# kabkabm/defensegan

Hardware: NVIDIA H100
Metric: reconstructed images/sec at R=10,L=200 (higher is better)
Workload: dtype f16

## Files before the change

defensegan_b200/csrc/dgan_api.cu:

```cuda
#include <algorithm>
#include <cmath>
#include <cstdio>
#include <cstring>
#include <functional>
#include <memory>
#include <new>

#include "common.cuh"
#include "kernels_simt.cuh"
#include "kernels_tc.cuh"
#include "kernels_tc2.cuh"
#include "kernels_vjp.cuh"
#include "kernels_measured.cuh"
#include "kernels_measured_csr.cuh"
#include "kernels_measured_conv.cuh"
#include "kernels_prune.cuh"
#include "kernels_adam.cuh"
#include "kernels_sparse_dev.cuh"

namespace dgan {

static thread_local std::string g_last_error;
void set_error(const std::string& msg) { g_last_error = msg; }

// ... 215 lines not shown
  int n_bands = 0;
  int n_blocks = 0;
  size_t fwd_smem = 0, bwd_smem = 0;
};

}

using namespace dgan;

struct dgan_ctx {
  dgan_desc desc;
  Widths wd{};
  int H = 0, W = 0, C = 0, hwc = 0;
  std::vector<GemmLayer> layers;
  FinalLayer fin;
  std::vector<void*> allocs;
  int64_t macs_per_row = 0;
  int64_t last_launches = 0;
  int64_t launches = 0;
  TcState tc;
  std::vector<TcDir> tc_dirs;
  std::vector<TcDir> tc_jvp_dirs;
  std::vector<TcDir> tc_w_dirs;
  bool profile = false;
  int n_rows_cur = 0;
  struct LoopGraph {
    const void* ws; int batch, rec_rr, rec_iters, decay_lr, weighted, measured, csr_nnz; float rec_lr, momentum;
    std::vector<int> prune;
    cudaGraphExec_t exec; int64_t kernels;
    int adam = 0; float beta1 = 0.f, beta2 = 0.f, eps = 0.f;
    float huber = 0.f;
    std::vector<int> conv;
    int prior = 0; float z_prior = 0.f;
    int sdev = 0; float sdev_l1 = 0.f, sdev_step = 0.f;
    bool same_key(const LoopGraph& o) const {
      return ws == o.ws && batch == o.batch && rec_rr == o.rec_rr && rec_iters == o.rec_iters && decay_lr == o.decay_lr &&
             weighted == o.weighted && measured == o.measured && csr_nnz == o.csr_nnz && rec_lr == o.rec_lr &&
             momentum == o.momentum && prune == o.prune && adam == o.adam && beta1 == o.beta1 && beta2 == o.beta2 &&
             eps == o.eps && huber == o.huber && conv == o.conv && prior == o.prior && z_prior == o.z_prior &&
             sdev == o.sdev && sdev_l1 == o.sdev_l1 && sdev_step == o.sdev_step;
    }
  };
  std::vector<LoopGraph> graphs;
  cudaStream_t cap_stream = nullptr;
  int64_t last_enqueues = 0;
  struct ProfRec { int kind; cudaEvent_t a, b; };
// ... 853 lines not shown
static int image_loss_finish(dgan_ctx* c, const Workspace& w, cudaStream_t s) {
  return loss_finish(c, w, w.loss_part, w.n_loss_parts, w.loss_stride_n, w.loss_stride_b, 1.0f / (float)c->hwc, s);
}

static int plan_all(dgan_ctx* c, int n_rows) {
  if (c->desc.precision != DGAN_PREC_FP16) return 0;
  const int n_mpairs = (int)align_up((size_t)std::max(n_rows, 1), 2 * kRowTile) / (2 * kRowTile);
  int rc;
  for (TcDir& t : c->tc_dirs)
    if ((rc = tc2_get_schedule(t, n_mpairs, c->tc.num_sms / 2, &c->allocs))) return rc;
  return 0;
}

static int plan_pass(dgan_ctx* c, int n_rows, TcPass pass) {
  if (c->desc.precision != DGAN_PREC_FP16) return 0;
  int rc;
  std::vector<TcDir>& have = pass == TC_PASS_TANGENT ? c->tc_jvp_dirs : c->tc_w_dirs;
  if (have.empty()) {
    std::vector<TcDir> dirs = tc_directions(&c->desc, pass);
    for (TcDir& t : dirs) {
      if ((rc = tc_dir_supported(t))) return rc;
      for (const TcDir& p : c->tc_dirs)
        if (p.ld == t.ld && p.col0 == t.col0) { t.w = p.w; t.tm_b = p.tm_b; }
    }
    have = std::move(dirs);
  }
  const int n_mpairs = (int)align_up((size_t)std::max(n_rows, 1), 2 * kRowTile) / (2 * kRowTile);
  for (TcDir& t : have)
    if ((rc = tc2_get_schedule(t, n_mpairs, c->tc.num_sms / 2, &c->allocs))) return rc;
  return 0;
}

static int check_ws(dgan_ctx* c, int n_rows, void* ws, size_t ws_bytes, Workspace* out, bool weighted = false, int m = 0,
                    int csr_nnz = -1, bool adam = false, const ConvGeom* conv = nullptr, bool sdev = false) {
  if (ws == nullptr) { set_error("workspace is NULL"); return DGAN_ERR_WORKSPACE; }
  if (((uintptr_t)ws & 1023) != 0) { set_error("workspace must be 1024-byte aligned"); return DGAN_ERR_WORKSPACE; }
  int rc;
  const bool wpass = weighted && !sdev;
  if ((rc = plan_all(c, n_rows))) return rc;
  if (wpass && (rc = plan_pass(c, n_rows, TC_PASS_WEIGHTED))) return rc;
  *out = carve(c, n_rows, ws, nullptr, weighted, m, csr_nnz, false, nullptr, adam, conv, sdev);
  if (out->bytes > ws_bytes) {
    set_error("workspace too small: need " + std::to_string(out->bytes) + " bytes, got " + std::to_string(ws_bytes) +
              (sdev ? (m > 0 ? " (dgan_workspace_bytes_measured_sparse_dev)" : " (dgan_workspace_bytes_sparse_dev)")
               : conv != nullptr ? " (dgan_workspace_bytes_measured_conv)"
               : adam ? (m > 0 ? " (dgan_workspace_bytes_measured_adam)" : " (dgan_workspace_bytes_adam)")
// ... 1412 lines not shown
    flops_per_launch_out[k] = 2.0 * h->kind_macs_per_row[k] * (double)h->n_rows_cur;
  }
  for (auto& r : h->prof) {
    DGAN_CUDA_CHECK(cudaEventSynchronize(r.b));
    float ms = 0.f;
    DGAN_CUDA_CHECK(cudaEventElapsedTime(&ms, r.a, r.b));
    if (r.kind >= 0 && r.kind < nk) { ms_out[r.kind] += ms; launches_out[r.kind]++; }
    cudaEventDestroy(r.a); cudaEventDestroy(r.b);
  }
  h->prof.clear();
  return DGAN_OK;
}

static int check_plans_impl(const dgan_desc* d, int n_rows, int n_pairs, int mutate, TcPass pass) {
  using namespace dgan;
  if (d == nullptr || n_rows <= 0 || n_pairs <= 0) { set_error("invalid argument"); return DGAN_ERR_INVALID_ARG; }
  const int n_pad = ((n_rows + 2 * kRowTile - 1) / (2 * kRowTile)) * 2 * kRowTile, n_mpairs = n_pad / (2 * kRowTile);
  Widths wd;
  if (int rc = padded_widths(d, &wd)) return rc;
  const std::string wide_target = pass == TC_PASS_TANGENT ? "Generator.3.jvp" : pass == TC_PASS_WEIGHTED ? "last.fwd.w" : "Generator.3.fwd";
  for (const TcDir& dr : tc_directions(d, pass)) {
    if (int rc = tc_dir_supported(dr)) return rc;
    Tc2Plan plan;
    int rc = tc2_plan(dr.N, dr.K, dr.tab, dr.h_grid, dr.w_grid, dr.max_acc, 0, dr.epi, dr.out_bytes, n_mpairs, n_pairs, &plan);
    if (rc) { set_error(dr.name + ": " + dgan_last_error()); return rc; }
    const bool narrow = (mutate == 12 || mutate == 13) && dr.name == "last.bwd";
    const bool wide = mutate != 0 && mutate != 12 && mutate != 13 && dr.name == wide_target;
    if ((narrow || wide) && plan.stream_m.size() > 40) {
      auto mma = [&](size_t i, auto f) { TcMmaRec m = TcMmaRec::decode(plan.stream_m[i]); f(m); plan.stream_m[i] = m.encode(); };
      auto producer = [&](size_t i, auto f) { TcProducerRec p = TcProducerRec::decode(plan.stream_p[i]); f(p); plan.stream_p[i] = p.encode(); };
      auto every_mma = [&](auto f) { for (size_t i = 0; i < plan.stream_m.size(); ++i) mma(i, f); };
      switch (mutate) {
        case 1: mma(20, [](TcMmaRec& m) {
                  TcOp op = TcOp::decode(m.ops[0]);
                  op.first ^= 1u;
                  m.ops[0] = op.encode();
                });
                break;
        case 2: mma(20, [](TcMmaRec& m) {
                  for (uint32_t j = 1; j < m.maxb; ++j)
                    if (m.ops[j] != m.ops[0]) { std::swap(m.ops[0], m.ops[j]); break; }
                });
                break;
        case 3: producer(20, [](TcProducerRec& p) { p.tile[0] ^= 1u; }); break;
        case 4: producer(20, [](TcProducerRec& p) { p.pix[0] ^= 1u; }); break;
        case 5: producer(20, [](TcProducerRec& p) { p.kc ^= 1u; }); break;
        case 6: plan.eitems[0] = -1; break;
// ... 12 lines not shown
        case 13: producer(20, [](TcProducerRec& p) { p.kc |= 1u; }); break;
        case 14: mma(20, [](TcMmaRec& m) {
                   for (uint32_t j = 0; j < m.maxb; ++j) m.ops[j] = TC2_PAD_OP;
                 });
                 break;
        case 15: {
                   bool done = false;
                   for (size_t i = 20; i < plan.stream_m.size() && !done; ++i)
                     mma(i, [&](TcMmaRec& m) {
                       for (uint32_t j = 0; j < m.n_rounds * m.maxb && !done; ++j)
                         if (TcOp::decode(m.ops[j]).slot == (uint32_t)TC2_ZERO_SLOT) {
                           m.ops[j] = (uint8_t)TcOp::First::put(m.ops[j], 1u);
                           done = true;
                         }
                     });
                   break;
                 }
        default: break;
      }
    }
    std::string err;
    if ((rc = tc2_check_plan(dr.N, dr.K, dr.tab, n_mpairs, dr.epi, dr.out_bytes, plan, &err))) { set_error(dr.name + ": " + err); return rc; }
    if (mutate != 0) continue;
    for (const Tc2Kind& k : kTc2Kinds) {
      if (k.n != dr.N || k.ksub != plan.ksub || k.epi != dr.epi || k.out_bytes != dr.out_bytes || k.maxb == plan.maxb) continue;
      Tc2Plan forced;
      if ((rc = tc2_plan(dr.N, dr.K, dr.tab, dr.h_grid, dr.w_grid, dr.max_acc, k.maxb, dr.epi, dr.out_bytes, n_mpairs, n_pairs, &forced))) {
        set_error(dr.name + " (" + std::to_string(k.maxb) + " slots): " + dgan_last_error());
        return rc;
      }
      if ((rc = tc2_check_plan(dr.N, dr.K, dr.tab, n_mpairs, dr.epi, dr.out_bytes, forced, &err))) {
        set_error(dr.name + " (" + std::to_string(k.maxb) + " slots): " + err);
        return rc;
      }
    }
  }
  return 0;
}

int dgan_debug_check_plans(const dgan_desc* d, int n_rows, int n_pairs, int mutate) {
  return check_plans_impl(d, n_rows, n_pairs, mutate, TC_PASS_PROJ);
}

int dgan_debug_check_tangent_plans(const dgan_desc* d, int n_rows, int n_pairs, int mutate) {
  return check_plans_impl(d, n_rows, n_pairs, mutate, TC_PASS_TANGENT);
}

int dgan_debug_check_weighted_plans(const dgan_desc* d, int n_rows, int n_pairs, int mutate) {
  return check_plans_impl(d, n_rows, n_pairs, mutate, TC_PASS_WEIGHTED);
}


int dgan_debug_force_slots(dgan_handle h, int dir, int maxb) {
  if (h == nullptr || h->desc.precision != DGAN_PREC_FP16 || maxb < 0) { set_error("invalid argument"); return DGAN_ERR_INVALID_ARG; }
  if (dir < 0 || dir >= (int)h->tc_dirs.size()) { set_error("layer-direction out of range"); return DGAN_ERR_INVALID_ARG; }
  TcDir& d = h->tc_dirs[(size_t)dir];
  if (maxb > 0 && !tc2_has_kind(d.N, maxb, tc2_ksub(d.K), d.epi, d.out_bytes)) {
    set_error("no kernel instantiation with " + std::to_string(maxb) + " accumulator slots per round for this layer-direction");
    return DGAN_ERR_UNSUPPORTED;
  }
  d.force_maxb = maxb;
  d.by_mpairs.clear();
  for (auto& g : h->graphs) cudaGraphExecDestroy(g.exec);
  h->graphs.clear();
  return DGAN_OK;
}

int dgan_debug_slot_choices(dgan_handle h, int dir, int* out, int max_n) {
  if (h == nullptr || h->desc.precision != DGAN_PREC_FP16 || out == nullptr) return -1;
  if (dir < 0 || dir >= (int)h->tc_dirs.size()) return -1;
  const TcDir& d = h->tc_dirs[(size_t)dir];
  int n = 0;
  for (const Tc2Kind& k : kTc2Kinds)
    if (k.n == d.N && k.ksub == tc2_ksub(d.K) && k.epi == d.epi && k.out_bytes == d.out_bytes && n < max_n) out[n++] = k.maxb;
  return n;
}

#ifdef DGAN_PROBE
int dgan_debug_probe_read(unsigned long long* out) {
  if (cudaDeviceSynchronize() != cudaSuccess) return -1;
  if (cudaMemcpyFromSymbol(out, dgan::g_tc2_probe, sizeof(dgan::g_tc2_probe)) != cudaSuccess) return -1;
  static unsigned long long zeros[48 * 160 * dgan::TC2_PROBE_WORDS];
  if (cudaMemcpyToSymbol(dgan::g_tc2_probe, zeros, sizeof(zeros)) != cudaSuccess) return -1;
  return 0;
}
// ... 6 lines not shown
  const int n_pad = ((n_rows + 2 * kRowTile - 1) / (2 * kRowTile)) * 2 * kRowTile, n_mpairs = n_pad / (2 * kRowTile);
  Widths wd;
  if (padded_widths(d, &wd) != 0) return -1;
  std::string out = "direction | N | K | window (h x w, stride) | items | slots | steps | MMAs | staged MB | busiest pair / mean load"
                    " | zero-tile MMA % | MMAs per round | busiest pair: est. tensor us | busiest pair: est. us | k16 MMAs"
                    " | epilogue/output\n";
  auto epi_name = [](int epi) {
    switch (epi) {
      case EPI_BIAS_RELU: return "bias_relu";
      case EPI_BIAS: return "bias";
      case EPI_MASK: return "mask";
      case EPI_FINAL_SIGMOID1: return "final_sigmoid";
      case EPI_FINAL_TANH3: return "final_tanh";
      default: return "none";
    }
  };
  double total = 0.0;
  const std::vector<TcDir> dirs = tc_directions(d);
  for (size_t di = 0; di < dirs.size(); ++di) {
    const TcDir& dr = dirs[di];
    Tc2Plan plan;
    const bool forced = (int)di == force_dir;
    const int rc = tc2_plan(dr.N, dr.K, dr.tab, dr.h_grid, dr.w_grid, dr.max_acc, forced ? force_maxb : 0, dr.epi, dr.out_bytes,
                            n_mpairs, n_pairs, &plan, forced ? force_shape : nullptr);
    if (rc) return -1;
    char line[320];
    const double mb = (double)plan.n_bytes / 1e6;
    total += mb;
    snprintf(line, sizeof line, "%s | %d | %d | %dx%d, %dx%d | %zu | %d | %lld | %lld | %.1f | %.3f | %.1f | %d | %.1f | %.1f | %lld | %s/f%d\n",
             dr.name.c_str(), dr.N, dr.K, plan.shape[0], plan.shape[1], plan.shape[2], plan.shape[3],
             plan.hdrs.size() * (size_t)n_mpairs, plan.n_slots, plan.n_steps, plan.n_mma, mb, plan.load_max / std::max(plan.load_mean, 1.0),
             100.0 * (double)plan.n_pad / (double)std::max(plan.n_mma, 1LL), plan.maxb, plan.op_ns_max / 1e3,
             plan.load_max / 1e3, plan.n_mma * plan.ksub, epi_name(dr.epi), 8 * dr.out_bytes);
    out += line;
  }
  char line[64];
  snprintf(line, sizeof line, "total staged MB per L-step | %.1f\n", total);
  out += line;
  const int n = (int)std::min(out.size(), (size_t)buf_len - 1);
  memcpy(buf, out.data(), (size_t)n);
  buf[n] = 0;
  return n;
}

int dgan_debug_plan_stats_slots(const dgan_desc* d, int n_rows, int n_pairs, int force_dir, int force_maxb, char* buf, int buf_len) {
  return plan_stats_impl(d, n_rows, n_pairs, force_dir, force_maxb, nullptr, buf, buf_len);
}

int dgan_debug_plan_stats_window(const dgan_desc* d, int n_rows, int n_pairs, int force_dir, int force_maxb, int wh, int ww,
                                 int sy, int sx, char* buf, int buf_len) {
  const int shape[4] = {wh, ww, sy, sx};
  return plan_stats_impl(d, n_rows, n_pairs, force_dir, force_maxb, shape, buf, buf_len);
}

int dgan_debug_plan_issue_stats(const dgan_desc* d, int n_rows, int n_pairs, char* buf, int buf_len) {
  using namespace dgan;
  if (d == nullptr || n_rows <= 0 || n_pairs <= 0 || buf == nullptr || buf_len <= 0) { set_error("invalid argument"); return -1; }
  const int n_pad = ((n_rows + 2 * kRowTile - 1) / (2 * kRowTile)) * 2 * kRowTile, n_mpairs = n_pad / (2 * kRowTile);
  Widths wd;
  if (padded_widths(d, &wd) != 0) return -1;
  std::string out = "direction | slots | k16 MMAs issued | zero-tile k16 MMAs skipped | busiest pair: est. tensor us, issued\n";
  for (const TcDir& dr : tc_directions(d)) {
    Tc2Plan plan;
    if (tc2_plan(dr.N, dr.K, dr.tab, dr.h_grid, dr.w_grid, dr.max_acc, 0, dr.epi, dr.out_bytes, n_mpairs, n_pairs, &plan)) return -1;
    char line[200];
    snprintf(line, sizeof line, "%s | %d | %lld | %lld | %.1f\n", dr.name.c_str(), plan.maxb, plan.n_issued * plan.ksub,
             (plan.n_mma - plan.n_issued) * plan.ksub, plan.op_ns_issued_max / 1e3);
    out += line;
  }
  const int n = (int)std::min(out.size(), (size_t)buf_len - 1);
  memcpy(buf, out.data(), (size_t)n);
  buf[n] = 0;
  return n;
}

int dgan_debug_padded_widths(const dgan_desc* d, int* out) {
  using namespace dgan;
  if (d == nullptr || out == nullptr) { set_error("invalid argument"); return DGAN_ERR_INVALID_ARG; }
  Widths w;
  if (int rc = padded_widths(d, &w)) return rc;
  out[0] = w.latent; out[1] = w.c4; out[2] = w.c2; out[3] = w.c1;
  return 0;
}

static int workspace_layout_impl(dgan_handle h, int n_rows, char* buf, int buf_len, bool weighted, int m = 0,
                                 int csr_nnz = -1) {
  if (h == nullptr || n_rows <= 0 || buf == nullptr || buf_len <= 0) { set_error("invalid argument"); return -1; }
// ... 109 lines not shown
```

defensegan_b200/csrc/kernels_tc2.cuh:

```cuda
#pragma once
#include "kernels_tc.cuh"
#include "tc_records.cuh"

namespace dgan {

constexpr int TC2_SMEM_MAX = 232448;
constexpr int TC2_TILE_BYTES = 128 * 128;
constexpr int TC2_BUF_COLS = 256;
constexpr int TC2_CONSUMERS = 256;
constexpr int TC2_THREADS = TC2_CONSUMERS + 128;
constexpr int TC2_PRODUCER_REGS = 40, TC2_CONSUMER_REGS = 232;
constexpr int TC2_STORE_ROWS = 16;

constexpr int TC2_MAX_PAIRS = 80;
struct Tc2Heads {
  uint32_t off[TC2_MAX_PAIRS + 1];
};

struct __align__(16) TcItem2 {
  uint16_t q[16];
  uint32_t n_acc;
};
static_assert(sizeof(TcItem2) == 48 && offsetof(TcItem2, n_acc) == 32, "the kernel's item loads");

// ... 819 lines not shown
      if (probe_steps != 0) atomicAdd(&g_tc2_probe[key][blockIdx.x][14], (unsigned long long)((unsigned)clock64() - probe_h0));
      atomicAdd(&g_tc2_probe[key][blockIdx.x][0], (unsigned long long)(clock64() - probe_t_go));
      atomicAdd(&g_tc2_probe[key][blockIdx.x][1], 1ull);
      atomicAdd(&g_tc2_probe[key][blockIdx.x][2], (unsigned long long)(probe_t_go - probe_t_entry));
      atomicAdd(&g_tc2_probe[key][blockIdx.x][4], (unsigned long long)(probe_t_entry - probe_t_start));
      g_tc2_probe[key][blockIdx.x][5] = probe_g_start;
      g_tc2_probe[key][blockIdx.x][6] = probe_gtime();
    }
  }
#endif
  ptx::cluster_sync();
}

struct Tc2Schedule {
  TcItem2* items = nullptr;
  TcRec* stream_p = nullptr;
  TcRec* stream_m = nullptr;
  Tc2Heads heads{};
  int* eitems = nullptr;
  int n_slots = 0, n_pairs = 0;
  int maxb = 1;
};
static uint32_t tc2_box_k(int K) { return tc2_ksub(K) == 4 ? 64u : 16u; }
struct TcDir {
  std::string name, kind;
  int N = 0, K = 0, P_in = 0, P_out = 0, n_tiles = 0;
  PairTable tab;
  int h_grid = 0, w_grid = 0;
  int max_acc = 1;
  int epi = EPI_NONE, out_bytes = 2, bias_pstride = 0;
  int ld = 0, col0 = 0, out_ld = 0;
  int n_real = 0;
  std::string base_kind;
  __half* w = nullptr;
  CUtensorMap tm_b{};
  int force_maxb = 0;
  std::vector<std::pair<int, Tc2Schedule>> by_mpairs;
};

static int tc2_maxb(int N) { return TC2_BUF_COLS / tc2_acc_stride(N); }

struct Tc2HostStep {
  int kc = 0, nA = 0, nB = 0, n_rounds = 0;
  int a_pix[TC2_MAX_A] = {0, 0, 0, 0};
  uint8_t b_ent[TC2_MAX_BSLOTS] = {0};
  uint8_t ops[TC2_OP_BYTES] = {0};
  int n_real = 0;
  int bytes = 0;
};
struct Tc2HostItem {
  TcItem2 hdr{};
  std::vector<Tc2HostStep> steps;
  double stage_bytes = 0.0;
  long long n_ops = 0;
  long long n_issued = 0;
};

static void tc2_build_item(const PairTable& tab, const std::vector<int>& qs, int N, int K, int max_b, int max_a,
                           int step_max_bytes, Tc2HostItem* out) {
// ... 125 lines not shown
#define DGAN_STEP_MAX_KB_N64 64
#endif
#ifndef DGAN_COST_EPI_KB
#define DGAN_COST_EPI_KB 24.0
#endif
#ifndef DGAN_COST_FIXED_KB
#define DGAN_COST_FIXED_KB 48.0
#endif
#ifndef DGAN_COST_NS_PER_KB
#define DGAN_COST_NS_PER_KB 6.8
#endif
#ifndef DGAN_COST_OP_NS
#define DGAN_COST_OP_NS 103.0
#endif
#ifndef DGAN_COST_STEP_NS
#define DGAN_COST_STEP_NS 942.0
#endif
#ifndef DGAN_COST_OP_MIN_N
#define DGAN_COST_OP_MIN_N 32
#endif
#ifndef TC2_REFINE_BUDGET
#define TC2_REFINE_BUDGET (1LL << 26)
#endif

struct Tc2Plan {
  int shape[4] = {1, 1, 1, 1};
  int n_slots = 0, n_pairs = 0;
  std::vector<TcItem2> hdrs;
  std::vector<TcRec> stream_p, stream_m;
  std::vector<uint32_t> stream_off;
  std::vector<int> eitems;
  long long n_mma = 0, n_pad = 0, n_issued = 0, n_steps = 0, n_bytes = 0;
  double load_max = 0.0, load_mean = 0.0;
  double op_ns_max = 0.0;
  double op_ns_issued_max = 0.0;
  int maxb = 1, ring_bytes = 0;
  int ksub = 4;
};

static double tc2_op_ns(int N, int ksub) {
  return DGAN_COST_OP_NS * (double)std::max(N, DGAN_COST_OP_MIN_N) / 64.0 * (double)ksub / 4.0;
}

static int tc2_search(int N, int K, const PairTable& tab, int h_grid, int w_grid, int max_acc, int force_maxb, int epi,
                      int out_bytes, int n_mpairs, int n_pairs, const int* force_shape, Tc2Plan* plan,
                      std::vector<Tc2HostItem>* best_items, std::vector<std::vector<int>>* best_lists) {
  const int max_a = TC2_MAX_A;
  const int step_kb = (N == 64 && K == 128) ? DGAN_STEP_MAX_KB_N64 : DGAN_STEP_MAX_KB;
  const int ksub = tc2_ksub(K);
  const double op_ns = tc2_op_ns(N, ksub);
  double best_cost = 1e300;
  plan->maxb = 0;
  std::vector<std::vector<int>> wins;
  for (const Tc2Kind& kind : kTc2Kinds) {
    if (kind.n != N || kind.ksub != ksub || kind.epi != epi || kind.out_bytes != out_bytes) continue;
    if (force_maxb > 0 && kind.maxb != force_maxb) continue;
    const int mb = kind.maxb, ring = tc2_ring_bytes(N, mb, ksub, epi, out_bytes);
    const int step_max = std::min((ring / 3) & ~1023, step_kb * 1024);
    for (int wh = 1; wh <= 2; ++wh)
      for (int ww = 1; ww <= 8; ++ww)
        for (int sy = 1; sy <= (wh > 1 ? 2 : 1); ++sy)
          for (int sx = 1; sx <= (ww > 1 ? 2 : 1); ++sx) {
            if (wh * ww > std::min(max_acc, mb) || wh > h_grid || ww > std::max(w_grid, 1)) continue;
            if (force_shape != nullptr && (wh != force_shape[0] || ww != force_shape[1] || sy != force_shape[2] || sx != force_shape[3])) continue;
            tc2_enumerate_windows(h_grid, std::max(w_grid, 1), wh, ww, sy, sx, &wins);
            std::vector<Tc2HostItem> items(wins.size());
            for (size_t i = 0; i < wins.size(); ++i) tc2_build_item(tab, wins[i], N, K, mb, max_a, step_max, &items[i]);
            std::vector<double> icost(items.size());
            auto cost_item = [&](const Tc2HostItem& it) {
              return DGAN_COST_NS_PER_KB / 1024.0 *
                         (it.stage_bytes + DGAN_COST_EPI_KB * 1024.0 * it.hdr.n_acc * std::max(1, N / 64) + DGAN_COST_FIXED_KB * 1024.0) +
                     op_ns * (double)it.n_ops + DGAN_COST_STEP_NS * (double)it.steps.size();
            };
            std::stable_sort(items.begin(), items.end(), [](const Tc2HostItem& l, const Tc2HostItem& r) { return l.stage_bytes > r.stage_bytes; });
            for (size_t i = 0; i < items.size(); ++i) icost[i] = cost_item(items[i]);
            const long long total = (long long)items.size() * n_mpairs;
            std::vector<double> load((size_t)n_pairs, 0.0);
            std::vector<std::vector<int>> lists((size_t)n_pairs);
            for (long long idx = 0; idx < total; ++idx) {
              size_t best = 0;
              for (size_t pr = 1; pr < (size_t)n_pairs; ++pr)
                if (load[pr] < load[best]) best = pr;
              load[best] += icost[(size_t)(idx / n_mpairs)];
              lists[best].push_back((int)idx);
            }
            auto cost_of = [&](int idx) { return icost[(size_t)(idx / n_mpairs)]; };
            long long work = 0;
            for (int iter = 0; iter < 4096 && work < TC2_REFINE_BUDGET; ++iter) {
              const size_t P = (size_t)(std::max_element(load.begin(), load.end()) - load.begin());
              double best_peak = load[P];
              size_t bq = P; int bi = -1, bj = -1;
              for (size_t Q = 0; Q < (size_t)n_pairs; ++Q) {
                if (Q == P) continue;
                work += (long long)lists[P].size() * (long long)(1 + lists[Q].size());
                for (size_t i = 0; i < lists[P].size(); ++i) {
                  const double ci = cost_of(lists[P][i]);
                  double peak = std::max(load[P] - ci, load[Q] + ci);
                  if (peak < best_peak - 1e-9) { best_peak = peak; bq = Q; bi = (int)i; bj = -1; }
                  for (size_t j = 0; j < lists[Q].size(); ++j) {
                    const double cj = cost_of(lists[Q][j]);
                    if (cj >= ci) continue;
                    peak = std::max(load[P] - ci + cj, load[Q] + ci - cj);
                    if (peak < best_peak - 1e-9) { best_peak = peak; bq = Q; bi = (int)i; bj = (int)j; }
                  }
                }
              }
              if (bi < 0) break;
              const int it_i = lists[P][(size_t)bi];
              const double ci = cost_of(it_i);
              if (bj < 0) {
                lists[P].erase(lists[P].begin() + bi);
                lists[bq].push_back(it_i);
                load[P] -= ci; load[bq] += ci;
              } else {
                const int it_j = lists[bq][(size_t)bj];
                const double cj = cost_of(it_j);
                lists[P][(size_t)bi] = it_j; lists[bq][(size_t)bj] = it_i;
                load[P] += cj - ci; load[bq] += ci - cj;
              }
            }
            for (auto& l : lists)
              std::stable_sort(l.begin(), l.end(), [&](int a, int b) { return cost_of(a) > cost_of(b); });
            const double makespan = *std::max_element(load.begin(), load.end());
            if (makespan < best_cost) {
              best_cost = makespan;
              plan->load_max = makespan;
              plan->load_mean = std::accumulate(load.begin(), load.end(), 0.0) / (double)n_pairs;
              plan->shape[0] = wh; plan->shape[1] = ww; plan->shape[2] = sy; plan->shape[3] = sx;
              plan->maxb = mb; plan->ring_bytes = ring;
              plan->op_ns_max = 0.0;
              plan->op_ns_issued_max = 0.0;
              for (size_t pr = 0; pr < lists.size(); ++pr)
                if (load[pr] == makespan) {
                  for (int idx : lists[pr]) {
                    plan->op_ns_max += op_ns * (double)items[(size_t)(idx / n_mpairs)].n_ops;
                    plan->op_ns_issued_max += op_ns * (double)items[(size_t)(idx / n_mpairs)].n_issued;
                  }
                  break;
                }
              best_items->swap(items); best_lists->swap(lists);
            }
          }
  }
  if (plan->maxb == 0) { set_error("no tensor-core kernel instantiation for this layer-direction"); return DGAN_ERR_UNSUPPORTED; }
  plan->ksub = ksub;
  return 0;
}

static int tc2_encode_streams(int N, int n_mpairs, int n_pairs, const std::vector<Tc2HostItem>& items,
                              const std::vector<std::vector<int>>& lists, Tc2Plan* plan) {
  const int max_b = plan->maxb, ring_bytes = plan->ring_bytes, ksub = plan->ksub;
  plan->n_pairs = n_pairs;
  size_t n_slots = 0;
  for (auto& l : lists) n_slots = std::max(n_slots, l.size());
  plan->n_slots = (int)n_slots;
  std::vector<int>& eitems = plan->eitems;
  eitems.assign(n_slots * (size_t)n_pairs, -1);
  std::vector<uint32_t>& stream_off = plan->stream_off;
  stream_off.assign((size_t)n_pairs + 1, 0);
  std::vector<TcRec>& stream_p = plan->stream_p;
  std::vector<TcRec>& stream_m = plan->stream_m;
  stream_p.clear(); stream_m.clear();
  long long n_mma = 0, n_pad = 0, n_issued = 0, n_steps = 0, n_bytes = 0;
  for (size_t pr = 0; pr < lists.size(); ++pr) {
    stream_off[pr] = (uint32_t)stream_m.size();
    std::vector<std::pair<int, int>> region;
    int cursor = 0;
    for (size_t k = 0; k < lists[pr].size(); ++k) {
      const int win = lists[pr][k] / n_mpairs, mp = lists[pr][k] % n_mpairs;
      if ((uint32_t)win > TcItemWindow::mask || (uint32_t)mp > TcItemMp::mask) { set_error("tensor-core schedule limits exceeded"); return DGAN_ERR_UNSUPPORTED; }
      eitems[k * (size_t)n_pairs + pr] = tc2_item_word(win, mp);
      const Tc2HostItem& itm = items[(size_t)win];
      for (size_t j = 0; j < itm.steps.size(); ++j) {
        const Tc2HostStep& hs = itm.steps[j];
        const int kb = (hs.bytes + 1023) / 1024;
        if (kb * 1024 > ring_bytes) { set_error("tensor-core step larger than the operand ring"); return DGAN_ERR_UNSUPPORTED; }
        if (cursor + kb > ring_bytes / 1024) cursor = 0;
        const int beg = cursor, end = cursor + kb;
        cursor = end;
        int dep = TC2_NSLOT;
        const int kidx = (int)region.size();
        for (int d = 1; d <= TC2_NSLOT && d <= kidx; ++d) {
          const auto& rg = region[(size_t)(kidx - d)];
          if (rg.first < end && beg < rg.second) { dep = d; break; }
        }
        if (dep == 1 && j > 0) { set_error("tensor-core step overlaps the step before it (ring too small)"); return DGAN_ERR_UNSUPPORTED; }
        region.push_back({beg, end});
        TcMmaRec m;
        m.off = (uint32_t)beg; m.nA = (uint32_t)hs.nA; m.n_rounds = (uint32_t)hs.n_rounds; m.maxb = (uint32_t)max_b; m.ksub = (uint32_t)ksub;
        m.flags = (j == 0 ? TcMmaRec::FIRST : 0u) | (j + 1 == itm.steps.size() ? TcMmaRec::LAST : 0u);
        std::copy(hs.ops, hs.ops + hs.n_rounds * max_b, m.ops);
        stream_m.push_back(m.encode());
        TcProducerRec p;
        p.off = (uint32_t)beg; p.kc = (uint32_t)hs.kc; p.nA = (uint32_t)hs.nA; p.nB = (uint32_t)hs.nB; p.dep = (uint32_t)dep; p.mp = (uint32_t)mp;
        std::copy(hs.a_pix, hs.a_pix + TC2_MAX_A, p.pix);
        std::copy(hs.b_ent, hs.b_ent + TC2_MAX_BSLOTS, p.tile);
        stream_p.push_back(p.encode());
        n_mma += hs.n_rounds * max_b; n_pad += hs.n_rounds * max_b - hs.n_real;
        n_issued += tc2_issues_zero_ops(max_b, ksub) ? hs.n_rounds * max_b : hs.n_real;
        n_steps += 1; n_bytes += 2LL * hs.nA * tc2_a_bytes(ksub) + (long long)hs.nB * tc2_b_bytes(N, ksub);
      }
    }
  }
  stream_off[(size_t)n_pairs] = (uint32_t)stream_m.size();
  plan->hdrs.resize(items.size());
  for (size_t i = 0; i < items.size(); ++i) plan->hdrs[i] = items[i].hdr;
  plan->n_mma = n_mma; plan->n_pad = n_pad; plan->n_issued = n_issued; plan->n_steps = n_steps; plan->n_bytes = n_bytes;
  return 0;
}

static int tc2_plan(int N, int K, const PairTable& tab, int h_grid, int w_grid, int max_acc, int force_maxb, int epi,
                    int out_bytes, int n_mpairs, int n_pairs, Tc2Plan* plan, const int* force_shape = nullptr) {
  std::vector<Tc2HostItem> items;
  std::vector<std::vector<int>> lists;
  const int rc = tc2_search(N, K, tab, h_grid, w_grid, max_acc, force_maxb, epi, out_bytes, n_mpairs, n_pairs, force_shape,
                            plan, &items, &lists);
  return rc ? rc : tc2_encode_streams(N, n_mpairs, n_pairs, items, lists, plan);
}

static int tc2_check_plan(int N, int K, const PairTable& tab, int n_mpairs, int epi, int out_bytes, const Tc2Plan& pl,
                          std::string* err) {
  auto fail = [&](const std::string& m) { *err = m; return DGAN_ERR_INVALID_ARG; };
  const int ksub = tc2_ksub(K), kch = K / (16 * ksub), a_bytes = tc2_a_bytes(ksub), b_tile = tc2_b_bytes(N, ksub);
  const int max_acc = pl.maxb;
  if (pl.ksub != ksub) return fail("plan's k16 MMAs per op disagree with the direction's channels");
  if (!tc2_has_kind(N, max_acc, ksub, epi, out_bytes)) return fail("no kernel instantiation with these accumulator slots per round");
  const int ring_bytes = tc2_ring_bytes(N, max_acc, ksub, epi, out_bytes);
  const size_t n_pairs = (size_t)pl.n_pairs;
  if (pl.stream_off.size() != n_pairs + 1) return fail("stream_off size");
  if (pl.stream_p.size() != pl.stream_m.size()) return fail("stream sizes differ");
  if (pl.eitems.size() != (size_t)pl.n_slots * n_pairs) return fail("eitems size");
  std::vector<int> assigned(pl.hdrs.size() * (size_t)n_mpairs, 0);
  for (const TcItem2& h : pl.hdrs) {
    if (h.n_acc < 1 || (int)h.n_acc > max_acc) return fail("window with too many accumulators");
    for (uint32_t a = 0; a < h.n_acc; ++a)
      if ((size_t)h.q[a] + 1 >= tab.off.size()) return fail("window pixel out of range");
  }
  struct Step { int beg, end; };
  for (size_t pr = 0; pr < n_pairs; ++pr) {
// ... 77 lines not shown
          for (int kc = 0; kc < kch; ++kc)
            for (int e2 = tab.off[hdr.q[a]]; e2 < tab.off[hdr.q[a] + 1]; ++e2) want.push_back({tab.pairs[e2].x * 32 + tab.pairs[e2].y, kc});
          std::vector<std::pair<int, int>> got = contrib[a];
          std::sort(want.begin(), want.end()); std::sort(got.begin(), got.end());
          if (want != got) return fail("an item's MMAs do not cover exactly its pair list");
        }
        in_item = false;
      }
    }
    if (in_item) return fail("stream ends inside an item");
    for (int kk = item_k + 1; kk < pl.n_slots; ++kk)
      if (pl.eitems[(size_t)kk * n_pairs + pr] != -1) return fail("epilogue list has an item the stream lacks");
  }
  for (int v : assigned)
    if (v != 1) return fail("an item is not assigned to any CTA pair");
  return 0;
}

static int tc2_get_schedule(TcDir& d, int n_mpairs, int n_pairs, std::vector<void*>* allocs) {
  for (auto& kv : d.by_mpairs)
    if (kv.first == n_mpairs) return 0;
  Tc2Plan plan;
  int rc;
  if ((rc = tc2_plan(d.N, d.K, d.tab, d.h_grid, d.w_grid, d.max_acc, d.force_maxb, d.epi, d.out_bytes, n_mpairs, n_pairs, &plan)))
    return rc;
  const cudaStream_t s = 0;
  Tc2Schedule sc;
  sc.maxb = plan.maxb;
  sc.n_pairs = n_pairs; sc.n_slots = plan.n_slots;
  if ((rc = tc_upload(allocs, plan.hdrs.data(), plan.hdrs.size() * sizeof(TcItem2), (void**)&sc.items, s))) return rc;
  if ((rc = tc_upload(allocs, plan.stream_p.data(), plan.stream_p.size() * sizeof(TcRec), (void**)&sc.stream_p, s))) return rc;
  if ((rc = tc_upload(allocs, plan.stream_m.data(), plan.stream_m.size() * sizeof(TcRec), (void**)&sc.stream_m, s))) return rc;
  if (n_pairs > TC2_MAX_PAIRS) { set_error("more CTA pairs than the kernel's parameter block holds"); return DGAN_ERR_UNSUPPORTED; }
  for (int pr = 0; pr <= n_pairs; ++pr) sc.heads.off[pr] = plan.stream_off[(size_t)pr];
  if ((rc = tc_upload(allocs, plan.eitems.data(), plan.eitems.size() * sizeof(int), (void**)&sc.eitems, s))) return rc;
  d.by_mpairs.push_back({n_mpairs, sc});
  return 0;
}

template <int NT, int MB, int KS, int EP, typename TOUT>
static cudaError_t tc2_optin() {
  return cudaFuncSetAttribute(tc_bsgemm2_kernel<NT, MB, KS, EP, TOUT>, cudaFuncAttributeMaxDynamicSharedMemorySize,
                              Tc2Cfg<NT, MB, KS, EP, (int)sizeof(TOUT)>::SMEM_BYTES);
}

static int tc2_optin_all() {
#define TC2_OPTIN(NT, MB, KS, EP, T) DGAN_CUDA_CHECK((tc2_optin<NT, MB, KS, EP, T>()));
// ... 36 lines not shown
```

Baseline: 2928.

## Order tensor-core work items in row bands to keep activations L2-resident

Adds a band ordering mode to the tensor-core scheduler. Work items are grouped by bands of row-tile pairs sized to fit a fixed L2 budget, and the band direction alternates between layers so a consumer starts on rows its producer just wrote. The band assignment is used only when its modeled makespan stays within a small tolerance of the LPT schedule and the input is large enough. It is meant to cut DRAM traffic for re-read activations, at the cost of slightly worse load balance and extra host-side planning.

```diff
diff --git a/defensegan_b200/csrc/dgan_api.cu b/defensegan_b200/csrc/dgan_api.cu
--- a/defensegan_b200/csrc/dgan_api.cu
+++ b/defensegan_b200/csrc/dgan_api.cu
@@ -261,6 +261,7 @@
   std::vector<TcDir> tc_dirs;
   std::vector<TcDir> tc_jvp_dirs;
   std::vector<TcDir> tc_w_dirs;
+  int tc_order = TC2_ORDER_BAND;
   bool profile = false;
   int n_rows_cur = 0;
   struct LoopGraph {
@@ -1160,6 +1161,7 @@
       if ((rc = tc_dir_supported(t))) return rc;
       for (const TcDir& p : c->tc_dirs)
         if (p.ld == t.ld && p.col0 == t.col0) { t.w = p.w; t.tm_b = p.tm_b; }
+      t.order = c->tc_order;
     }
     have = std::move(dirs);
   }
@@ -2618,7 +2620,9 @@
   for (const TcDir& dr : tc_directions(d, pass)) {
     if (int rc = tc_dir_supported(dr)) return rc;
     Tc2Plan plan;
-    int rc = tc2_plan(dr.N, dr.K, dr.tab, dr.h_grid, dr.w_grid, dr.max_acc, 0, dr.epi, dr.out_bytes, n_mpairs, n_pairs, &plan);
+    const bool rev = tc2_band_reverse(dr.ld);
+    int rc = tc2_plan(dr.N, dr.K, dr.tab, dr.h_grid, dr.w_grid, dr.max_acc, 0, dr.epi, dr.out_bytes, n_mpairs, n_pairs,
+                      dr.order, rev, &plan);
     if (rc) { set_error(dr.name + ": " + dgan_last_error()); return rc; }
     const bool narrow = (mutate == 12 || mutate == 13) && dr.name == "last.bwd";
     const bool wide = mutate != 0 && mutate != 12 && mutate != 13 && dr.name == wide_target;
@@ -2677,10 +2681,21 @@
     std::string err;
     if ((rc = tc2_check_plan(dr.N, dr.K, dr.tab, n_mpairs, dr.epi, dr.out_bytes, plan, &err))) { set_error(dr.name + ": " + err); return rc; }
     if (mutate != 0) continue;
+    Tc2Plan lpt;
+    if ((rc = tc2_plan(dr.N, dr.K, dr.tab, dr.h_grid, dr.w_grid, dr.max_acc, 0, dr.epi, dr.out_bytes, n_mpairs, n_pairs,
+                       TC2_ORDER_LPT, rev, &lpt))) {
+      set_error(dr.name + " (LPT order): " + dgan_last_error());
+      return rc;
+    }
+    if ((rc = tc2_check_plan(dr.N, dr.K, dr.tab, n_mpairs, dr.epi, dr.out_bytes, lpt, &err))) {
+      set_error(dr.name + " (LPT order): " + err);
+      return rc;
+    }
     for (const Tc2Kind& k : kTc2Kinds) {
       if (k.n != dr.N || k.ksub != plan.ksub || k.epi != dr.epi || k.out_bytes != dr.out_bytes || k.maxb == plan.maxb) continue;
       Tc2Plan forced;
-      if ((rc = tc2_plan(dr.N, dr.K, dr.tab, dr.h_grid, dr.w_grid, dr.max_acc, k.maxb, dr.epi, dr.out_bytes, n_mpairs, n_pairs, &forced))) {
+      if ((rc = tc2_plan(dr.N, dr.K, dr.tab, dr.h_grid, dr.w_grid, dr.max_acc, k.maxb, dr.epi, dr.out_bytes, n_mpairs, n_pairs,
+                         dr.order, rev, &forced))) {
         set_error(dr.name + " (" + std::to_string(k.maxb) + " slots): " + dgan_last_error());
         return rc;
       }
@@ -2716,6 +2731,22 @@
   }
   d.force_maxb = maxb;
   d.by_mpairs.clear();
+  for (auto& g : h->graphs) cudaGraphExecDestroy(g.exec);
+  h->graphs.clear();
+  return DGAN_OK;
+}
+
+int dgan_debug_force_order(dgan_handle h, int order) {
+  if (h == nullptr || h->desc.precision != DGAN_PREC_FP16 || (order != TC2_ORDER_LPT && order != TC2_ORDER_BAND)) {
+    set_error("invalid argument");
+    return DGAN_ERR_INVALID_ARG;
+  }
+  h->tc_order = order;
+  for (std::vector<TcDir>* dirs : {&h->tc_dirs, &h->tc_jvp_dirs, &h->tc_w_dirs})
+    for (TcDir& d : *dirs) {
+      d.order = order;
+      d.by_mpairs.clear();
+    }
   for (auto& g : h->graphs) cudaGraphExecDestroy(g.exec);
   h->graphs.clear();
   return DGAN_OK;
@@ -2768,7 +2799,7 @@
     Tc2Plan plan;
     const bool forced = (int)di == force_dir;
     const int rc = tc2_plan(dr.N, dr.K, dr.tab, dr.h_grid, dr.w_grid, dr.max_acc, forced ? force_maxb : 0, dr.epi, dr.out_bytes,
-                            n_mpairs, n_pairs, &plan, forced ? force_shape : nullptr);
+                            n_mpairs, n_pairs, dr.order, tc2_band_reverse(dr.ld), &plan, forced ? force_shape : nullptr);
     if (rc) return -1;
     char line[320];
     const double mb = (double)plan.n_bytes / 1e6;
@@ -2799,6 +2830,36 @@
   return plan_stats_impl(d, n_rows, n_pairs, force_dir, force_maxb, shape, buf, buf_len);
 }
 
+int dgan_debug_plan_order_stats(const dgan_desc* d, int n_rows, int n_pairs, int order, char* buf, int buf_len) {
+  using namespace dgan;
+  if (d == nullptr || n_rows <= 0 || n_pairs <= 0 || buf == nullptr || buf_len <= 0 ||
+      (order != TC2_ORDER_LPT && order != TC2_ORDER_BAND)) {
+    set_error("invalid argument");
+    return -1;
+  }
+  const int n_pad = ((n_rows + 2 * kRowTile - 1) / (2 * kRowTile)) * 2 * kRowTile, n_mpairs = n_pad / (2 * kRowTile);
+  Widths wd;
+  if (padded_widths(d, &wd) != 0) return -1;
+  std::string out = "direction | order | band row pairs | busiest pair: LPT us | busiest pair: order us | staged A MB"
+                    " | staged weight MB | unique input MB | working set MB\n";
+  for (const TcDir& dr : tc_directions(d)) {
+    Tc2Plan plan;
+    if (tc2_plan(dr.N, dr.K, dr.tab, dr.h_grid, dr.w_grid, dr.max_acc, 0, dr.epi, dr.out_bytes, n_mpairs, n_pairs, order,
+                 tc2_band_reverse(dr.ld), &plan))
+      return -1;
+    char line[240];
+    snprintf(line, sizeof line, "%s | %s | %d | %.1f | %.1f | %.1f | %.1f | %.1f | %.1f\n", dr.name.c_str(),
+             plan.order == TC2_ORDER_BAND ? (tc2_band_reverse(dr.ld) ? "band-" : "band+") : "lpt", plan.band_rows,
+             plan.load_max / 1e3, plan.load_max_order / 1e3, plan.n_bytes_a / 1e6, plan.n_bytes_b / 1e6,
+             plan.uniq_a_bytes / 1e6, plan.ws_a_bytes / 1e6);
+    out += line;
+  }
+  const int n = (int)std::min(out.size(), (size_t)buf_len - 1);
+  memcpy(buf, out.data(), (size_t)n);
+  buf[n] = 0;
+  return n;
+}
+
 int dgan_debug_plan_issue_stats(const dgan_desc* d, int n_rows, int n_pairs, char* buf, int buf_len) {
   using namespace dgan;
   if (d == nullptr || n_rows <= 0 || n_pairs <= 0 || buf == nullptr || buf_len <= 0) { set_error("invalid argument"); return -1; }
@@ -2808,7 +2869,9 @@
   std::string out = "direction | slots | k16 MMAs issued | zero-tile k16 MMAs skipped | busiest pair: est. tensor us, issued\n";
   for (const TcDir& dr : tc_directions(d)) {
     Tc2Plan plan;
-    if (tc2_plan(dr.N, dr.K, dr.tab, dr.h_grid, dr.w_grid, dr.max_acc, 0, dr.epi, dr.out_bytes, n_mpairs, n_pairs, &plan)) return -1;
+    if (tc2_plan(dr.N, dr.K, dr.tab, dr.h_grid, dr.w_grid, dr.max_acc, 0, dr.epi, dr.out_bytes, n_mpairs, n_pairs, dr.order,
+                 tc2_band_reverse(dr.ld), &plan))
+      return -1;
     char line[200];
     snprintf(line, sizeof line, "%s | %d | %lld | %lld | %.1f\n", dr.name.c_str(), plan.maxb, plan.n_issued * plan.ksub,
              (plan.n_mma - plan.n_issued) * plan.ksub, plan.op_ns_issued_max / 1e3);
diff --git a/defensegan_b200/csrc/kernels_tc2.cuh b/defensegan_b200/csrc/kernels_tc2.cuh
--- a/defensegan_b200/csrc/kernels_tc2.cuh
+++ b/defensegan_b200/csrc/kernels_tc2.cuh
@@ -1,4 +1,6 @@
 #pragma once
+#include <unordered_map>
+
 #include "kernels_tc.cuh"
 #include "tc_records.cuh"
 
@@ -865,6 +867,7 @@
   int maxb = 1;
 };
 static uint32_t tc2_box_k(int K) { return tc2_ksub(K) == 4 ? 64u : 16u; }
+enum Tc2Order { TC2_ORDER_LPT = 0, TC2_ORDER_BAND = 1 };
 struct TcDir {
   std::string name, kind;
   int N = 0, K = 0, P_in = 0, P_out = 0, n_tiles = 0;
@@ -878,6 +881,7 @@
   __half* w = nullptr;
   CUtensorMap tm_b{};
   int force_maxb = 0;
+  int order = TC2_ORDER_BAND;
   std::vector<std::pair<int, Tc2Schedule>> by_mpairs;
 };
 
@@ -1049,6 +1053,15 @@
 #ifndef TC2_REFINE_BUDGET
 #define TC2_REFINE_BUDGET (1LL << 26)
 #endif
+#ifndef TC2_BAND_L2_BYTES
+#define TC2_BAND_L2_BYTES (16 << 20)
+#endif
+#ifndef TC2_BAND_TOLERANCE
+#define TC2_BAND_TOLERANCE 0.02
+#endif
+#ifndef TC2_BAND_MIN_INPUT
+#define TC2_BAND_MIN_INPUT (9 << 20)
+#endif
 
 struct Tc2Plan {
   int shape[4] = {1, 1, 1, 1};
@@ -1058,9 +1071,14 @@
   std::vector<uint32_t> stream_off;
   std::vector<int> eitems;
   long long n_mma = 0, n_pad = 0, n_issued = 0, n_steps = 0, n_bytes = 0;
+  long long n_bytes_a = 0, n_bytes_b = 0;
+  long long uniq_a_bytes = 0;
+  long long ws_a_bytes = 0;
   double load_max = 0.0, load_mean = 0.0;
   double op_ns_max = 0.0;
   double op_ns_issued_max = 0.0;
+  int order = TC2_ORDER_LPT, band_rows = 0;
+  double load_max_order = 0.0;
   int maxb = 1, ring_bytes = 0;
   int ksub = 4;
 };
@@ -1069,9 +1087,84 @@
   return DGAN_COST_OP_NS * (double)std::max(N, DGAN_COST_OP_MIN_N) / 64.0 * (double)ksub / 4.0;
 }
 
+static double tc2_item_cost(const Tc2HostItem& it, int N, double op_ns) {
+  return DGAN_COST_NS_PER_KB / 1024.0 *
+             (it.stage_bytes + DGAN_COST_EPI_KB * 1024.0 * it.hdr.n_acc * std::max(1, N / 64) + DGAN_COST_FIXED_KB * 1024.0) +
+         op_ns * (double)it.n_ops + DGAN_COST_STEP_NS * (double)it.steps.size();
+}
+
+static int tc2_band_of(int idx, int n_mpairs, int band_rows, bool reverse) {
+  const int b = (idx % n_mpairs) / band_rows, n_bands = (n_mpairs + band_rows - 1) / band_rows;
+  return reverse ? n_bands - 1 - b : b;
+}
+
+static double tc2_assign(const std::vector<double>& icost, int n_mpairs, int n_pairs, int band_rows, bool reverse,
+                         size_t max_items, std::vector<std::vector<int>>* lists_out, std::vector<double>* load_out) {
+  const long long total = (long long)icost.size() * n_mpairs;
+  auto cost_of = [&](int idx) { return icost[(size_t)(idx / n_mpairs)]; };
+  auto band_of = [&](int idx) { return band_rows > 0 ? tc2_band_of(idx, n_mpairs, band_rows, reverse) : 0; };
+  std::vector<int> seq((size_t)total);
+  std::iota(seq.begin(), seq.end(), 0);
+  if (band_rows > 0)
+    std::stable_sort(seq.begin(), seq.end(), [&](int a, int b) {
+      return band_of(a) != band_of(b) ? band_of(a) < band_of(b) : cost_of(a) > cost_of(b);
+    });
+  std::vector<double>& load = *load_out;
+  std::vector<std::vector<int>>& lists = *lists_out;
+  load.assign((size_t)n_pairs, 0.0);
+  lists.assign((size_t)n_pairs, {});
+  const size_t cap = max_items > 0 ? max_items : (size_t)total;
+  for (int idx : seq) {
+    size_t best = (size_t)n_pairs;
+    for (size_t pr = 0; pr < (size_t)n_pairs; ++pr)
+      if (lists[pr].size() < cap && (best == (size_t)n_pairs || load[pr] < load[best])) best = pr;
+    load[best] += cost_of(idx);
+    lists[best].push_back(idx);
+  }
+  long long work = 0;
+  for (int iter = 0; iter < 4096 && work < TC2_REFINE_BUDGET; ++iter) {
+    const size_t P = (size_t)(std::max_element(load.begin(), load.end()) - load.begin());
+    double best_peak = load[P];
+    size_t bq = P; int bi = -1, bj = -1;
+    for (size_t Q = 0; Q < (size_t)n_pairs; ++Q) {
+      if (Q == P) continue;
+      work += (long long)lists[P].size() * (long long)(1 + lists[Q].size());
+      for (size_t i = 0; i < lists[P].size(); ++i) {
+        const double ci = cost_of(lists[P][i]);
+        double peak = std::max(load[P] - ci, load[Q] + ci);
+        if (lists[Q].size() < cap && peak < best_peak - 1e-9) { best_peak = peak; bq = Q; bi = (int)i; bj = -1; }
+        for (size_t j = 0; j < lists[Q].size(); ++j) {
+          const double cj = cost_of(lists[Q][j]);
+          if (cj >= ci || band_of(lists[Q][j]) != band_of(lists[P][i])) continue;
+          peak = std::max(load[P] - ci + cj, load[Q] + ci - cj);
+          if (peak < best_peak - 1e-9) { best_peak = peak; bq = Q; bi = (int)i; bj = (int)j; }
+        }
+      }
+    }
+    if (bi < 0) break;
+    const int it_i = lists[P][(size_t)bi];
+    const double ci = cost_of(it_i);
+    if (bj < 0) {
+      lists[P].erase(lists[P].begin() + bi);
+      lists[bq].push_back(it_i);
+      load[P] -= ci; load[bq] += ci;
+    } else {
+      const int it_j = lists[bq][(size_t)bj];
+      const double cj = cost_of(it_j);
+      lists[P][(size_t)bi] = it_j; lists[bq][(size_t)bj] = it_i;
+      load[P] += cj - ci; load[bq] += ci - cj;
+    }
+  }
+  for (auto& l : lists)
+    std::stable_sort(l.begin(), l.end(), [&](int a, int b) {
+      return band_of(a) != band_of(b) ? band_of(a) < band_of(b) : cost_of(a) > cost_of(b);
+    });
+  return *std::max_element(load.begin(), load.end());
+}
+
 static int tc2_search(int N, int K, const PairTable& tab, int h_grid, int w_grid, int max_acc, int force_maxb, int epi,
-                      int out_bytes, int n_mpairs, int n_pairs, const int* force_shape, Tc2Plan* plan,
-                      std::vector<Tc2HostItem>* best_items, std::vector<std::vector<int>>* best_lists) {
+                      int out_bytes, int n_mpairs, int n_pairs, int order, bool reverse, const int* force_shape,
+                      Tc2Plan* plan, std::vector<Tc2HostItem>* best_items, std::vector<std::vector<int>>* best_lists) {
   const int max_a = TC2_MAX_A;
   const int step_kb = (N == 64 && K == 128) ? DGAN_STEP_MAX_KB_N64 : DGAN_STEP_MAX_KB;
   const int ksub = tc2_ksub(K);
@@ -1079,6 +1172,7 @@
   double best_cost = 1e300;
   plan->maxb = 0;
   std::vector<std::vector<int>> wins;
+  std::vector<double> best_load;
   for (const Tc2Kind& kind : kTc2Kinds) {
     if (kind.n != N || kind.ksub != ksub || kind.epi != epi || kind.out_bytes != out_bytes) continue;
     if (force_maxb > 0 && kind.maxb != force_maxb) continue;
@@ -1093,84 +1187,68 @@
             tc2_enumerate_windows(h_grid, std::max(w_grid, 1), wh, ww, sy, sx, &wins);
             std::vector<Tc2HostItem> items(wins.size());
             for (size_t i = 0; i < wins.size(); ++i) tc2_build_item(tab, wins[i], N, K, mb, max_a, step_max, &items[i]);
+            std::stable_sort(items.begin(), items.end(), [](const Tc2HostItem& l, const Tc2HostItem& r) { return l.stage_bytes > r.stage_bytes; });
             std::vector<double> icost(items.size());
-            auto cost_item = [&](const Tc2HostItem& it) {
-              return DGAN_COST_NS_PER_KB / 1024.0 *
-                         (it.stage_bytes + DGAN_COST_EPI_KB * 1024.0 * it.hdr.n_acc * std::max(1, N / 64) + DGAN_COST_FIXED_KB * 1024.0) +
-                     op_ns * (double)it.n_ops + DGAN_COST_STEP_NS * (double)it.steps.size();
-            };
-            std::stable_sort(items.begin(), items.end(), [](const Tc2HostItem& l, const Tc2HostItem& r) { return l.stage_bytes > r.stage_bytes; });
-            for (size_t i = 0; i < items.size(); ++i) icost[i] = cost_item(items[i]);
-            const long long total = (long long)items.size() * n_mpairs;
-            std::vector<double> load((size_t)n_pairs, 0.0);
-            std::vector<std::vector<int>> lists((size_t)n_pairs);
-            for (long long idx = 0; idx < total; ++idx) {
-              size_t best = 0;
-              for (size_t pr = 1; pr < (size_t)n_pairs; ++pr)
-                if (load[pr] < load[best]) best = pr;
-              load[best] += icost[(size_t)(idx / n_mpairs)];
-              lists[best].push_back((int)idx);
-            }
-            auto cost_of = [&](int idx) { return icost[(size_t)(idx / n_mpairs)]; };
-            long long work = 0;
-            for (int iter = 0; iter < 4096 && work < TC2_REFINE_BUDGET; ++iter) {
-              const size_t P = (size_t)(std::max_element(load.begin(), load.end()) - load.begin());
-              double best_peak = load[P];
-              size_t bq = P; int bi = -1, bj = -1;
-              for (size_t Q = 0; Q < (size_t)n_pairs; ++Q) {
-                if (Q == P) continue;
-                work += (long long)lists[P].size() * (long long)(1 + lists[Q].size());
-                for (size_t i = 0; i < lists[P].size(); ++i) {
-                  const double ci = cost_of(lists[P][i]);
-                  double peak = std::max(load[P] - ci, load[Q] + ci);
-                  if (peak < best_peak - 1e-9) { best_peak = peak; bq = Q; bi = (int)i; bj = -1; }
-                  for (size_t j = 0; j < lists[Q].size(); ++j) {
-                    const double cj = cost_of(lists[Q][j]);
-                    if (cj >= ci) continue;
-                    peak = std::max(load[P] - ci + cj, load[Q] + ci - cj);
-                    if (peak < best_peak - 1e-9) { best_peak = peak; bq = Q; bi = (int)i; bj = (int)j; }
-                  }
-                }
-              }
-              if (bi < 0) break;
-              const int it_i = lists[P][(size_t)bi];
-              const double ci = cost_of(it_i);
-              if (bj < 0) {
-                lists[P].erase(lists[P].begin() + bi);
-                lists[bq].push_back(it_i);
-                load[P] -= ci; load[bq] += ci;
-              } else {
-                const int it_j = lists[bq][(size_t)bj];
-                const double cj = cost_of(it_j);
-                lists[P][(size_t)bi] = it_j; lists[bq][(size_t)bj] = it_i;
-                load[P] += cj - ci; load[bq] += ci - cj;
-              }
-            }
-            for (auto& l : lists)
-              std::stable_sort(l.begin(), l.end(), [&](int a, int b) { return cost_of(a) > cost_of(b); });
-            const double makespan = *std::max_element(load.begin(), load.end());
+            for (size_t i = 0; i < items.size(); ++i) icost[i] = tc2_item_cost(items[i], N, op_ns);
+            std::vector<std::vector<int>> lists;
+            std::vector<double> load;
+            const double makespan = tc2_assign(icost, n_mpairs, n_pairs, 0, false, 0, &lists, &load);
             if (makespan < best_cost) {
               best_cost = makespan;
-              plan->load_max = makespan;
-              plan->load_mean = std::accumulate(load.begin(), load.end(), 0.0) / (double)n_pairs;
               plan->shape[0] = wh; plan->shape[1] = ww; plan->shape[2] = sy; plan->shape[3] = sx;
               plan->maxb = mb; plan->ring_bytes = ring;
-              plan->op_ns_max = 0.0;
-              plan->op_ns_issued_max = 0.0;
-              for (size_t pr = 0; pr < lists.size(); ++pr)
-                if (load[pr] == makespan) {
-                  for (int idx : lists[pr]) {
-                    plan->op_ns_max += op_ns * (double)items[(size_t)(idx / n_mpairs)].n_ops;
-                    plan->op_ns_issued_max += op_ns * (double)items[(size_t)(idx / n_mpairs)].n_issued;
-                  }
-                  break;
-                }
-              best_items->swap(items); best_lists->swap(lists);
+              best_items->swap(items); best_lists->swap(lists); best_load.swap(load);
             }
           }
   }
   if (plan->maxb == 0) { set_error("no tensor-core kernel instantiation for this layer-direction"); return DGAN_ERR_UNSUPPORTED; }
   plan->ksub = ksub;
+  const std::vector<Tc2HostItem>& items = *best_items;
+  plan->load_max = best_cost;
+  plan->load_mean = std::accumulate(best_load.begin(), best_load.end(), 0.0) / (double)n_pairs;
+  plan->op_ns_max = 0.0;
+  plan->op_ns_issued_max = 0.0;
+  for (size_t pr = 0; pr < best_lists->size(); ++pr)
+    if (best_load[pr] == best_cost) {
+      for (int idx : (*best_lists)[pr]) {
+        plan->op_ns_max += op_ns * (double)items[(size_t)(idx / n_mpairs)].n_ops;
+        plan->op_ns_issued_max += op_ns * (double)items[(size_t)(idx / n_mpairs)].n_issued;
+      }
+      break;
+    }
+  plan->order = TC2_ORDER_LPT;
+  plan->band_rows = 0;
+  plan->load_max_order = best_cost;
+  std::vector<double> icost(items.size());
+  for (size_t i = 0; i < items.size(); ++i) icost[i] = tc2_item_cost(items[i], N, op_ns);
+  if (order == TC2_ORDER_BAND && n_mpairs > 1) {
+    std::vector<int> pix;
+    long long n_out = 0;
+    for (const Tc2HostItem& it : items) {
+      n_out += it.hdr.n_acc;
+      for (const Tc2HostStep& st : it.steps) pix.insert(pix.end(), st.a_pix, st.a_pix + st.nA);
+    }
+    std::sort(pix.begin(), pix.end());
+    const long long n_in = std::unique(pix.begin(), pix.end()) - pix.begin();
+    const long long mp_bytes = 2LL * kRowTile * (2LL * K * n_in + (long long)out_bytes * N * n_out);
+    const int fill = (n_pairs + (int)items.size() - 1) / (int)items.size();
+    const int fit = (int)std::max(1LL, (long long)TC2_BAND_L2_BYTES / std::max(mp_bytes, 1LL));
+    const int band_rows = std::min(n_mpairs, std::max(1, std::min(fill, fit)));
+    const long long in_bytes = 2LL * kRowTile * n_mpairs * 2LL * K * n_in;
+    if (band_rows < n_mpairs && in_bytes >= (long long)TC2_BAND_MIN_INPUT) {
+      std::vector<std::vector<int>> lists;
+      std::vector<double> load;
+      size_t lpt_items = 0;
+      for (const auto& l : *best_lists) lpt_items = std::max(lpt_items, l.size());
+      const double makespan = tc2_assign(icost, n_mpairs, n_pairs, band_rows, reverse, lpt_items, &lists, &load);
+      if (makespan <= best_cost * (1.0 + TC2_BAND_TOLERANCE)) {
+        plan->order = TC2_ORDER_BAND;
+        plan->band_rows = band_rows;
+        plan->load_max_order = makespan;
+        best_lists->swap(lists);
+      }
+    }
+  }
   return 0;
 }
 
@@ -1188,9 +1266,12 @@
   std::vector<TcRec>& stream_p = plan->stream_p;
   std::vector<TcRec>& stream_m = plan->stream_m;
   stream_p.clear(); stream_m.clear();
-  long long n_mma = 0, n_pad = 0, n_issued = 0, n_steps = 0, n_bytes = 0;
+  long long n_mma = 0, n_pad = 0, n_issued = 0, n_steps = 0, n_bytes_a = 0, n_bytes_b = 0;
+  const double op_ns = tc2_op_ns(N, ksub);
+  std::unordered_map<long long, std::pair<double, double>> a_span;
   for (size_t pr = 0; pr < lists.size(); ++pr) {
     stream_off[pr] = (uint32_t)stream_m.size();
+    double t_item = 0.0;
     std::vector<std::pair<int, int>> region;
     int cursor = 0;
     for (size_t k = 0; k < lists[pr].size(); ++k) {
@@ -1198,8 +1279,15 @@
       if ((uint32_t)win > TcItemWindow::mask || (uint32_t)mp > TcItemMp::mask) { set_error("tensor-core schedule limits exceeded"); return DGAN_ERR_UNSUPPORTED; }
       eitems[k * (size_t)n_pairs + pr] = tc2_item_word(win, mp);
       const Tc2HostItem& itm = items[(size_t)win];
+      const double c_item = tc2_item_cost(itm, N, op_ns);
       for (size_t j = 0; j < itm.steps.size(); ++j) {
         const Tc2HostStep& hs = itm.steps[j];
+        const double t = t_item + c_item * (double)j / (double)itm.steps.size();
+        for (int a = 0; a < hs.nA; ++a) {
+          const long long key = ((long long)mp * 16 + hs.kc) * 65536 + hs.a_pix[a];
+          auto ins = a_span.insert({key, {t, t}});
+          if (!ins.second) ins.first->second.second = t;
+        }
         const int kb = (hs.bytes + 1023) / 1024;
         if (kb * 1024 > ring_bytes) { set_error("tensor-core step larger than the operand ring"); return DGAN_ERR_UNSUPPORTED; }
         if (cursor + kb > ring_bytes / 1024) cursor = 0;
@@ -1225,23 +1313,35 @@
         stream_p.push_back(p.encode());
         n_mma += hs.n_rounds * max_b; n_pad += hs.n_rounds * max_b - hs.n_real;
         n_issued += tc2_issues_zero_ops(max_b, ksub) ? hs.n_rounds * max_b : hs.n_real;
-        n_steps += 1; n_bytes += 2LL * hs.nA * tc2_a_bytes(ksub) + (long long)hs.nB * tc2_b_bytes(N, ksub);
-      }
-    }
-  }
+        n_steps += 1; n_bytes_a += 2LL * hs.nA * tc2_a_bytes(ksub); n_bytes_b += (long long)hs.nB * tc2_b_bytes(N, ksub);
+      }
+      t_item += c_item;
+    }
+  }
+  std::vector<std::pair<double, int>> ev;
+  for (const auto& kv : a_span) { ev.push_back({kv.second.first, 1}); ev.push_back({kv.second.second, -1}); }
+  std::sort(ev.begin(), ev.end(), [](const auto& l, const auto& r) { return l.first != r.first ? l.first < r.first : l.second > r.second; });
+  long long live = 0, peak = 0;
+  for (const auto& e : ev) { live += e.second; peak = std::max(peak, live); }
+  plan->uniq_a_bytes = 2LL * tc2_a_bytes(ksub) * (long long)a_span.size();
+  plan->ws_a_bytes = 2LL * tc2_a_bytes(ksub) * peak;
   stream_off[(size_t)n_pairs] = (uint32_t)stream_m.size();
   plan->hdrs.resize(items.size());
   for (size_t i = 0; i < items.size(); ++i) plan->hdrs[i] = items[i].hdr;
-  plan->n_mma = n_mma; plan->n_pad = n_pad; plan->n_issued = n_issued; plan->n_steps = n_steps; plan->n_bytes = n_bytes;
+  plan->n_mma = n_mma; plan->n_pad = n_pad; plan->n_issued = n_issued; plan->n_steps = n_steps;
+  plan->n_bytes_a = n_bytes_a; plan->n_bytes_b = n_bytes_b; plan->n_bytes = n_bytes_a + n_bytes_b;
   return 0;
 }
 
+static bool tc2_band_reverse(int ld) { return (((ld >> 1) + (ld & 1)) & 1) != 0; }
+
 static int tc2_plan(int N, int K, const PairTable& tab, int h_grid, int w_grid, int max_acc, int force_maxb, int epi,
-                    int out_bytes, int n_mpairs, int n_pairs, Tc2Plan* plan, const int* force_shape = nullptr) {
+                    int out_bytes, int n_mpairs, int n_pairs, int order, bool reverse, Tc2Plan* plan,
+                    const int* force_shape = nullptr) {
   std::vector<Tc2HostItem> items;
   std::vector<std::vector<int>> lists;
-  const int rc = tc2_search(N, K, tab, h_grid, w_grid, max_acc, force_maxb, epi, out_bytes, n_mpairs, n_pairs, force_shape,
-                            plan, &items, &lists);
+  const int rc = tc2_search(N, K, tab, h_grid, w_grid, max_acc, force_maxb, epi, out_bytes, n_mpairs, n_pairs, order,
+                            reverse, force_shape, plan, &items, &lists);
   return rc ? rc : tc2_encode_streams(N, n_mpairs, n_pairs, items, lists, plan);
 }
 
@@ -1365,7 +1465,8 @@
     if (kv.first == n_mpairs) return 0;
   Tc2Plan plan;
   int rc;
-  if ((rc = tc2_plan(d.N, d.K, d.tab, d.h_grid, d.w_grid, d.max_acc, d.force_maxb, d.epi, d.out_bytes, n_mpairs, n_pairs, &plan)))
+  if ((rc = tc2_plan(d.N, d.K, d.tab, d.h_grid, d.w_grid, d.max_acc, d.force_maxb, d.epi, d.out_bytes, n_mpairs, n_pairs,
+                     d.order, tc2_band_reverse(d.ld), &plan)))
     return rc;
   const cudaStream_t s = 0;
   Tc2Schedule sc;
```

New measurement: 3053, median of 6. 4.3% higher.
